# jayleicn/TVRetrieval

Hardware: AMD Instinct MI355X
Metric: queries/sec VCMR over 21.8K-video corpus (higher is better)
Workload: dtype bf16

## Files before the change

tvretrieval_amd/csrc/convse.hip:

```cpp
#include "band.h"
#include "gemm.h"

static constexpr int TM = 64;
static constexpr int LP = 128 + 8;
static constexpr int LH = 4;

static constexpr int CONVSE_SUB_MAX = 16;
static inline int convse_sub(int64_t P, int nv) { return P >= 128 * (int64_t)nv ? CONVSE_SUB_MAX : 1; }

struct ConvseWs {
  int32_t* counts;
  int32_t* offsets;
  int32_t* pos;
  int32_t* chunk_off;
  int32_t* bucket;
  int32_t* chunk_vid;
};

static size_t convse_ws_layout(const xml_convse_desc* d, ConvseWs* w, char* base) {
  size_t off = 0;
  auto take = [&](size_t bytes) {
    char* p = base ? base + off : nullptr;
    off += align_up(bytes, 256);
    return p;
  };
  const size_t nv = (size_t)d->nv, P = (size_t)d->nq * d->kpairs;
  char* counts = take(nv * CONVSE_SUB_MAX * 4);
  char* offsets = take((nv * CONVSE_SUB_MAX + 1) * 4);
  char* chunk_off = take((nv + 1) * 4);
  char* bucket = take(P * 4);
  char* pos = take(P * 4);
  char* chunk_vid = take((P / TM + (P < nv ? P : nv) + 1) * 4);
  if (w) {
    w->chunk_vid = (int32_t*)chunk_vid;
    w->counts = (int32_t*)counts; w->pos = (int32_t*)pos; w->offsets = (int32_t*)offsets;
    w->chunk_off = (int32_t*)chunk_off; w->bucket = (int32_t*)bucket;
  }
  return off;
}

extern "C" size_t xml_convse_rerank_workspace_bytes(const xml_convse_desc* d) {
  if (!d) return 0;
  return convse_ws_layout(d, nullptr, nullptr);
}

__global__ void convse_count_kernel(const int32_t* __restrict__ pair_vid, int32_t* __restrict__ counts,
                                    int32_t* __restrict__ pos, int64_t P, int nv, int sub) {
  const int64_t p = (int64_t)blockIdx.x * blockDim.x + threadIdx.x;
  if (p >= P) return;
  const int v = pair_vid[p];
  pos[p] = (v >= 0 && v < nv) ? atomicAdd(&counts[(int64_t)v * sub + (int)(p & (sub - 1))], 1) : -1;
}

__global__ void convse_zero_skipped_kernel(const int32_t* __restrict__ pair_vid, float* __restrict__ st_out,
                                           float* __restrict__ ed_out, int64_t P, int nv, int lpad4) {
  const int64_t p = (int64_t)blockIdx.x * blockDim.x + threadIdx.x;
  if (p >= P) return;
  const int v = pair_vid[p];
  if (v >= 0 && v < nv) return;
  const float4 z = make_float4(0.f, 0.f, 0.f, 0.f);
  float4* s4 = reinterpret_cast<float4*>(st_out) + p * lpad4;
  float4* e4 = reinterpret_cast<float4*>(ed_out) + p * lpad4;
  for (int i = 0; i < lpad4; ++i) { s4[i] = z; e4[i] = z; }
}

__global__ __launch_bounds__(1024) void convse_scan_kernel(const int32_t* __restrict__ counts,
                                                           int32_t* __restrict__ offsets,
                                                           int32_t* __restrict__ chunk_off,
                                                           int32_t* __restrict__ chunk_vid, int nv, int TM, int sub) {
  __shared__ int32_t wa[16], wb[16];
  const int tid = threadIdx.x, lane = tid & 63, wave = tid >> 6;
  const int per = (nv + 1023) / 1024;
  const int r0 = min(nv, tid * per), r1 = min(nv, r0 + per);
  int sa = 0, sb = 0;
  for (int i = r0; i < r1; ++i) {
    int c = 0;
    for (int j = 0; j < sub; ++j) c += counts[(int64_t)i * sub + j];
    sa += c; sb += (c + TM - 1) / TM;
  }
  int ia = sa, ib = sb;
#pragma unroll
  for (int o = 1; o < 64; o <<= 1) {
    const int va = __shfl_up(ia, o, 64), vb = __shfl_up(ib, o, 64);
    if (lane >= o) { ia += va; ib += vb; }
  }
  if (lane == 63) { wa[wave] = ia; wb[wave] = ib; }
  __syncthreads();
  int a = ia - sa, b = ib - sb;
  for (int w = 0; w < wave; ++w) { a += wa[w]; b += wb[w]; }
  for (int i = r0; i < r1; ++i) {
    int c = 0;
    for (int j = 0; j < sub; ++j) {
      const int cj = counts[(int64_t)i * sub + j];
      offsets[(int64_t)i * sub + j] = a + c;
      c += cj;
    }
    const int ch = (c + TM - 1) / TM;
    chunk_off[i] = b;
    for (int j = 0; j < ch; ++j) chunk_vid[b + j] = i;
    a += c; b += ch;
  }
  if (tid == 1023) { offsets[(int64_t)nv * sub] = a; chunk_off[nv] = b; }
}

__global__ void convse_fill_kernel(const int32_t* __restrict__ pair_vid, const int32_t* __restrict__ offsets,
                                   const int32_t* __restrict__ pos, int32_t* __restrict__ bucket, int64_t P, int sub) {
  const int64_t p = (int64_t)blockIdx.x * blockDim.x + threadIdx.x;
  if (p >= P) return;
  const int r = pos[p];
  if (r >= 0) bucket[offsets[(int64_t)pair_vid[p] * sub + (int)(p & (sub - 1))] + r] = (int32_t)p;
}

static constexpr int CONVSE_SMALL_NV = 4096, CONVSE_SMALL_P = 32768;
__global__ __launch_bounds__(1024) void convse_invert_small_kernel(const int32_t* __restrict__ pair_vid,
                                                                   int32_t* __restrict__ offsets, int32_t* __restrict__ chunk_off,
                                                                   int32_t* __restrict__ chunk_vid, int32_t* __restrict__ pos,
                                                                   int32_t* __restrict__ bucket, float* __restrict__ st_out,
                                                                   float* __restrict__ ed_out, int P, int nv, int TM, int lpad4,
                                                                   int zero_skipped) {
  __shared__ int32_t s_cnt[CONVSE_SMALL_NV], s_off[CONVSE_SMALL_NV];
  __shared__ int32_t wa[16], wb[16];
  const int tid = threadIdx.x, lane = tid & 63, wave = tid >> 6;
  for (int i = tid; i < nv; i += 1024) s_cnt[i] = 0;
  const bool in_regs = P <= 8 * 1024;
  int v_r[8], pos_r[8];
#pragma unroll
  for (int j = 0; j < 8; ++j) {
    const int p = tid + j * 1024;
    v_r[j] = (in_regs && p < P) ? pair_vid[p] : -1;
  }
  __syncthreads();
  if (in_regs) {
#pragma unroll
    for (int j = 0; j < 8; ++j) {
      const int p = tid + j * 1024;
      const bool ok = v_r[j] >= 0 && v_r[j] < nv;
      pos_r[j] = ok ? atomicAdd(&s_cnt[v_r[j]], 1) : -1;
      if (p < P && !ok && zero_skipped) {
        const float4 z = make_float4(0.f, 0.f, 0.f, 0.f);
        float4* s4 = reinterpret_cast<float4*>(st_out) + (int64_t)p * lpad4;
        float4* e4 = reinterpret_cast<float4*>(ed_out) + (int64_t)p * lpad4;
        for (int i = 0; i < lpad4; ++i) { s4[i] = z; e4[i] = z; }
      }
    }
  } else {
  for (int p = tid; p < P; p += 1024) {
    const int v = pair_vid[p];
    const bool ok = v >= 0 && v < nv;
    pos[p] = ok ? atomicAdd(&s_cnt[v], 1) : -1;
    if (!ok && zero_skipped) {
      const float4 z = make_float4(0.f, 0.f, 0.f, 0.f);
      float4* s4 = reinterpret_cast<float4*>(st_out) + (int64_t)p * lpad4;
      float4* e4 = reinterpret_cast<float4*>(ed_out) + (int64_t)p * lpad4;
      for (int i = 0; i < lpad4; ++i) { s4[i] = z; e4[i] = z; }
    }
  }
  }
  __syncthreads();
  const int per = (nv + 1023) / 1024;
  const int r0 = min(nv, tid * per), r1 = min(nv, r0 + per);
// ... 503 lines not shown
  if (d->n_mod < 1 || d->n_mod > 2 || (d->n_mod == 2 && (!q_lin1 || !feat2_1))) return XML_ERR_BAD_ARG;
  if (d->n_mod == 2 && !d->merged && !mask1) return XML_ERR_BAD_ARG;
  if (d->merged && d->n_mod != 2) return XML_ERR_BAD_ARG;
  if (d->lpad % 16 || d->lpad > 128 || d->l_ref > d->lpad || d->l_ref <= 0 || d->hidden % 8) return XML_ERR_UNSUPPORTED;
  if (!(d->ksize & 1) || d->ksize > 15 || d->ksize < 1) return XML_ERR_UNSUPPORTED;
  if (d->dt != XML_F32 && d->dt != XML_BF16) return XML_ERR_BAD_ARG;
  return convse_rerank_impl(d, q_lin0, q_lin1, feat2_0, feat2_1, mask0, mask1, pair_vid, conv_w, st_out, ed_out, ws, ws_bytes,
                            nullptr, nullptr, nullptr, nullptr, stream);
}

extern "C" int xml_convse_rerank_f16s(const xml_convse_desc* d, const void* q_lin0, const void* q_lin1, const float* q_inv0,
                                      const float* q_inv1, const void* feat2_0, const void* feat2_1, const float* c_inv0,
                                      const float* c_inv1, const float* mask0, const float* mask1, const int32_t* pair_vid,
                                      const float* conv_w, float* st_out, float* ed_out, void* ws, size_t ws_bytes,
                                      xml_stream_t stream) {
  XML_ENTER();
  if (!d || !q_lin0 || !feat2_0 || !mask0 || !pair_vid || !conv_w || !st_out || !ed_out || !ws || !q_inv0 || !c_inv0)
    return XML_ERR_BAD_ARG;
  if (d->nq <= 0 || d->nv <= 0 || d->kpairs <= 0 || d->hidden <= 0) return XML_ERR_BAD_ARG;
  if (d->n_mod < 1 || d->n_mod > 2 || (d->n_mod == 2 && (!q_lin1 || !feat2_1 || !q_inv1 || !c_inv1))) return XML_ERR_BAD_ARG;
  if (d->n_mod == 2 && !d->merged && !mask1) return XML_ERR_BAD_ARG;
  if (d->merged && d->n_mod != 2) return XML_ERR_BAD_ARG;
  if (d->lpad % 16 || d->lpad > 128 || d->l_ref > d->lpad || d->l_ref <= 0 || d->hidden % 32) return XML_ERR_UNSUPPORTED;
  if (!(d->ksize & 1) || d->ksize > 15 || d->ksize < 1) return XML_ERR_UNSUPPORTED;
  if (d->dt != XML_F16S) return XML_ERR_BAD_ARG;
  return convse_rerank_impl(d, q_lin0, q_lin1, feat2_0, feat2_1, mask0, mask1, pair_vid, conv_w, st_out, ed_out, ws, ws_bytes,
                            q_inv0, q_inv1, c_inv0, c_inv1, stream);
}

static int convse_rerank_impl(const xml_convse_desc* d, const void* q_lin0, const void* q_lin1, const void* feat2_0,
                              const void* feat2_1, const float* mask0, const float* mask1, const int32_t* pair_vid,
                              const float* conv_w, float* st_out, float* ed_out, void* ws, size_t ws_bytes,
                              const float* q_inv0, const float* q_inv1, const float* c_inv0, const float* c_inv1,
                              xml_stream_t stream, ConvseSumm sm, ConvseEv ev) {
  xml_convse_desc dl = *d;
  if (ev.pair_q) { dl.nq = (int)ev.n_pairs; dl.kpairs = 1; }
  if (!ev.pair_q && ws_bytes < xml_convse_rerank_workspace_bytes(d)) return XML_ERR_WORKSPACE;
  hipStream_t st = (hipStream_t)stream;
  ConvseWs w;
  convse_ws_layout(&dl, &w, (char*)ws);
  const int64_t P = (int64_t)dl.nq * dl.kpairs;
  int sub = 1;
  if (P <= CONVSE_SMALL_P && d->nv <= CONVSE_SMALL_NV) {
    hipLaunchKernelGGL(convse_invert_small_kernel, dim3(1), dim3(1024), 0, st, pair_vid, w.offsets, w.chunk_off, w.chunk_vid,
                       w.pos, w.bucket, st_out, ed_out, (int)P, d->nv, TM, d->lpad / 4, (d->softmax & 2) ? 0 : 1);
    XML_CHECK_LAUNCH();
  } else {
    {
      const int64_t nwords = (int64_t)((char*)w.offsets - (char*)w.counts) / 4;
      hipLaunchKernelGGL(convse_zero_words_kernel, dim3(cdiv(nwords, 256)), dim3(256), 0, st, (uint32_t*)w.counts, nwords);
      XML_CHECK_LAUNCH();
    }
    sub = convse_sub(P, d->nv);
    hipLaunchKernelGGL(convse_count_kernel, dim3(cdiv(P, 256)), dim3(256), 0, st, pair_vid, w.counts, w.pos, P, d->nv, sub);
    XML_CHECK_LAUNCH();
    if (!(d->softmax & 2)) {
      hipLaunchKernelGGL(convse_zero_skipped_kernel, dim3(cdiv(P, 256)), dim3(256), 0, st, pair_vid, st_out, ed_out, P,
                         d->nv, d->lpad / 4);
      XML_CHECK_LAUNCH();
    }
    hipLaunchKernelGGL(convse_scan_kernel, dim3(1), dim3(1024), 0, st, w.counts, w.offsets, w.chunk_off, w.chunk_vid,
                       d->nv, TM, sub);
    XML_CHECK_LAUNCH();
    hipLaunchKernelGGL(convse_fill_kernel, dim3(cdiv(P, 256)), dim3(256), 0, st, pair_vid, w.offsets, w.pos, w.bucket, P, sub);
    XML_CHECK_LAUNCH();
  }
  ConvseArgs a;
  a.sub = sub;
  a.q_lin[0] = q_lin0; a.q_lin[1] = q_lin1;
  a.feat2[0] = feat2_0; a.feat2[1] = feat2_1;
  a.mask[0] = mask0; a.mask[1] = mask1 ? mask1 : mask0;
  a.conv_w = conv_w; a.st_out = st_out; a.ed_out = ed_out;
  a.offsets = w.offsets; a.chunk_off = w.chunk_off; a.bucket = w.bucket; a.chunk_vid = w.chunk_vid;
  a.pair_q = ev.pair_q; a.ev_sim[0] = ev.sim[0]; a.ev_sim[1] = ev.sim[1]; a.ev_merged = ev.merged;
  a.nv = d->nv; a.kpairs = dl.kpairs; a.lpad = d->lpad; a.l_ref = d->l_ref; a.hidden = d->hidden;
  a.n_mod = d->n_mod; a.merged = d->merged; a.ksize = d->ksize; a.softmax = d->softmax & 1;
  a.dbg = g_q2c_ablation;
  a.pair_w = sm.pair_w; a.summ = sm.summ; a.min_l = sm.min_l; a.max_l = sm.max_l; a.vid_len = sm.vid_len;
  a.q_inv[0] = q_inv0; a.q_inv[1] = q_inv1 ? q_inv1 : q_inv0;
  a.c_inv[0] = c_inv0; a.c_inv[1] = c_inv1 ? c_inv1 : c_inv0;
  {
    const int64_t kb = (int64_t)d->hidden * (int64_t)dt_size(d->dt);
    a.dma = (kb % 128 == 0 && (int64_t)d->nq * kb < (1ll << 32) && (int64_t)d->lpad * kb < (1ll << 32)) ? 1 : 0;
    if (g_q2c_ablation == 40) a.dma = 0;
  }
  const int64_t max_chunks = P / TM + (P < d->nv ? P : d->nv);
  const int n_sim = d->merged ? 1 : d->n_mod;
  const size_t patch = (size_t)TM * LP * 4;
  if (d->dt == XML_F16S) {
    if (!a.dma) return XML_ERR_UNSUPPORTED;
    using Cfg = GemmCfg<f16s_t, TM, 128, 1, 4>;
    constexpr size_t stg = Cfg::LDS_BYTES;
    const size_t lds = n_sim == 1 ? (stg > patch ? stg : patch) : stg + 2 * patch;
    if (ev.pair_q) {
      if (!xml_lds_attr_once<convse_kernel<f16s_t, true>>((int)(stg + 2 * patch))) return XML_ERR_LAUNCH;
      hipLaunchKernelGGL((convse_kernel<f16s_t, true>), dim3((unsigned)max_chunks), dim3(256), lds, st, a);
    } else {
      if (!xml_lds_attr_once<convse_kernel<f16s_t>>((int)(stg + 2 * patch))) return XML_ERR_LAUNCH;
      hipLaunchKernelGGL(convse_kernel<f16s_t>, dim3((unsigned)max_chunks), dim3(256), lds, st, a);
    }
  } else if (d->dt == XML_F32) {
    using Cfg = GemmCfg<float, TM, 128, 1, 4>;
    constexpr size_t stg = Cfg::LDS_BYTES;
    const size_t lds = n_sim == 1 ? (stg > patch ? stg : patch) : stg + 2 * patch;
    if (ev.pair_q) {
      if (!xml_lds_attr_once<convse_kernel<float, true>>((int)(stg + 2 * patch))) return XML_ERR_LAUNCH;
      hipLaunchKernelGGL((convse_kernel<float, true>), dim3((unsigned)max_chunks), dim3(256), lds, st, a);
    } else {
      if (!xml_lds_attr_once<convse_kernel<float>>((int)(stg + 2 * patch))) return XML_ERR_LAUNCH;
      hipLaunchKernelGGL(convse_kernel<float>, dim3((unsigned)max_chunks), dim3(256), lds, st, a);
    }
  } else {
    using Cfg = GemmCfg<bf16_t, TM, 128, 1, 4>;
    constexpr size_t stg = Cfg::LDS_BYTES;
    const size_t lds = n_sim == 1 ? (stg > patch ? stg : patch) : stg + 2 * patch;
    if (ev.pair_q) {
      if (!xml_lds_attr_once<convse_kernel<bf16_t, true>>((int)(stg + 2 * patch))) return XML_ERR_LAUNCH;
// ... 53 lines not shown
  }
  size_t vid_off = 0;
  if (ws_bytes < evidence_ws_layout(d, n_pairs, &vid_off)) return XML_ERR_WORKSPACE;
  hipStream_t st = (hipStream_t)stream;
  int32_t* vid_ok = (int32_t*)((char*)ws + vid_off);
  hipLaunchKernelGGL(evidence_pairs_kernel, dim3(cdiv(n_pairs, 256)), dim3(256), 0, st, pair_q, pair_vid, vid_ok, n_pairs,
                     d->nq, d->nv);
  XML_CHECK_LAUNCH();
  hipLaunchKernelGGL(convse_zero_skipped_kernel, dim3(cdiv(n_pairs, 256)), dim3(256), 0, st, vid_ok, sim0_out, sim_out,
                     n_pairs, d->nv, d->lpad / 4);
  XML_CHECK_LAUNCH();
  if (d->n_mod == 2) {
    hipLaunchKernelGGL(convse_zero_skipped_kernel, dim3(cdiv(n_pairs, 256)), dim3(256), 0, st, vid_ok, sim1_out, sim1_out,
                       n_pairs, d->nv, d->lpad / 4);
    XML_CHECK_LAUNCH();
  }
  xml_convse_desc dd = *d;
  dd.softmax = 0;
  return convse_rerank_impl(&dd, q_lin0, q_lin1, feat2_0, feat2_1, mask0, mask1, vid_ok, conv_w, st_out, ed_out, ws, ws_bytes,
                            split ? q_inv0 : nullptr, split ? q_inv1 : nullptr, split ? c_inv0 : nullptr,
                            split ? c_inv1 : nullptr, stream, ConvseSumm{nullptr, nullptr, 0, 0, nullptr},
                            ConvseEv{pair_q, n_pairs, {sim0_out, d->n_mod == 2 ? sim1_out : nullptr}, sim_out});
}

extern "C" size_t xml_q2c_rescore_workspace_bytes(int nq, int nv, int kpairs) {
  xml_convse_desc d{};
  d.nq = nq; d.nv = nv; d.kpairs = kpairs;
  return convse_ws_layout(&d, nullptr, nullptr);
}

extern "C" int xml_q2c_rescore(int n_mod, const void* qn0, const void* qn1, const void* cn0, const void* cn1,
                               const float* mask0, const float* mask1, const int32_t* pair_vid, float* out, int nq, int nv,
                               int kpairs, int lpad, int hidden, int dt, void* ws, size_t ws_bytes, xml_stream_t stream) {
  XML_ENTER();
  if (!qn0 || !cn0 || !mask0 || !pair_vid || !out || !ws) return XML_ERR_BAD_ARG;
  if (n_mod < 1 || n_mod > 2 || (n_mod == 2 && (!qn1 || !cn1 || !mask1))) return XML_ERR_BAD_ARG;
  if (nq <= 0 || nv <= 0 || kpairs <= 0 || hidden <= 0) return XML_ERR_BAD_ARG;
  if (lpad % 16 || lpad > 128 || lpad <= 0 || hidden % 8) return XML_ERR_UNSUPPORTED;
  if (dt != XML_F32 && dt != XML_BF16 && dt != XML_F16S) return XML_ERR_BAD_ARG;
  if (dt == XML_F16S && hidden % 32) return XML_ERR_UNSUPPORTED;
  if (ws_bytes < xml_q2c_rescore_workspace_bytes(nq, nv, kpairs)) return XML_ERR_WORKSPACE;
  hipStream_t st = (hipStream_t)stream;
  xml_convse_desc d{};
  d.nq = nq; d.nv = nv; d.kpairs = kpairs;
  ConvseWs w;
  convse_ws_layout(&d, &w, (char*)ws);
  const int64_t P = (int64_t)nq * kpairs;
  {
    const int64_t nwords = (int64_t)((char*)w.offsets - (char*)w.counts) / 4;
    hipLaunchKernelGGL(convse_zero_words_kernel, dim3(cdiv(nwords, 256)), dim3(256), 0, st, (uint32_t*)w.counts, nwords);
    XML_CHECK_LAUNCH();
  }
  const int sub = convse_sub(P, nv);
  hipLaunchKernelGGL(convse_count_kernel, dim3(cdiv(P, 256)), dim3(256), 0, st, pair_vid, w.counts, w.pos, P, nv, sub);
  XML_CHECK_LAUNCH();
  hipLaunchKernelGGL(rescore_fill_skipped_kernel, dim3(cdiv(P, 256)), dim3(256), 0, st, pair_vid, out, P, nv);
  XML_CHECK_LAUNCH();
  const bool big = dt == XML_F16S && P > 64 * (int64_t)nv;
  hipLaunchKernelGGL(convse_scan_kernel, dim3(1), dim3(1024), 0, st, w.counts, w.offsets, w.chunk_off, w.chunk_vid, nv,
                     big ? 128 : TM, sub);
  XML_CHECK_LAUNCH();
  hipLaunchKernelGGL(convse_fill_kernel, dim3(cdiv(P, 256)), dim3(256), 0, st, pair_vid, w.offsets, w.pos, w.bucket, P, sub);
  XML_CHECK_LAUNCH();
  RescoreArgs a;
  a.sub = sub;
  a.qn[0] = qn0; a.qn[1] = qn1; a.cn[0] = cn0; a.cn[1] = cn1;
  a.mask[0] = mask0; a.mask[1] = mask1 ? mask1 : mask0;
  a.out = out;
  a.offsets = w.offsets; a.chunk_off = w.chunk_off; a.bucket = w.bucket; a.chunk_vid = w.chunk_vid;
  a.nv = nv; a.kpairs = kpairs; a.lpad = lpad; a.hidden = hidden; a.n_mod = n_mod;
  {
    const int64_t kb = (int64_t)hidden * (int64_t)dt_size(dt);
    a.dma = (kb % 128 == 0 && (int64_t)nq * kb < (1ll << 32) && (int64_t)lpad * kb < (1ll << 32)) ? 1 : 0;
    if (g_q2c_ablation == 40) a.dma = 0;
  }
  const int64_t max_chunks = P / TM + (P < nv ? P : nv);
  if (dt == XML_F16S && big) {
    if (!a.dma) return XML_ERR_UNSUPPORTED;
    using Cfg = GemmCfg<f16s_t, 128, 128, 1, 4>;
    constexpr int lds = GemmDma<Cfg, RS_STAGES>::LDS_BYTES;
    if (!xml_lds_attr_once<rescore_kernel<f16s_t, 128>>(lds)) return XML_ERR_LAUNCH;
    const int64_t chunks128 = P / 128 + (P < nv ? P : nv);
    hipLaunchKernelGGL((rescore_kernel<f16s_t, 128>), dim3((unsigned)chunks128), dim3(256), lds, st, a);
  } else if (dt == XML_F16S) {
    using Cfg = GemmCfg<f16s_t, TM, 128, 1, 4>;
    constexpr int lds = GemmDma<Cfg, RS_STAGES>::LDS_BYTES;
    if (!xml_lds_attr_once<rescore_kernel<f16s_t>>(lds)) return XML_ERR_LAUNCH;
    hipLaunchKernelGGL(rescore_kernel<f16s_t>, dim3((unsigned)max_chunks), dim3(256), lds, st, a);
  } else if (dt == XML_F32) {
    using Cfg = GemmCfg<float, TM, 128, 1, 4>;
    constexpr int lds = GemmDma<Cfg, RS_STAGES>::LDS_BYTES;
    if (!xml_lds_attr_once<rescore_kernel<float>>(lds)) return XML_ERR_LAUNCH;
    hipLaunchKernelGGL(rescore_kernel<float>, dim3((unsigned)max_chunks), dim3(256), lds, st, a);
  } else {
    using Cfg = GemmCfg<bf16_t, TM, 128, 1, 4>;
    constexpr int lds = GemmDma<Cfg, RS_STAGES>::LDS_BYTES;
    if (!xml_lds_attr_once<rescore_kernel<bf16_t>>(lds)) return XML_ERR_LAUNCH;
    hipLaunchKernelGGL(rescore_kernel<bf16_t>, dim3((unsigned)max_chunks), dim3(256), lds, st, a);
  }
  XML_CHECK_LAUNCH();
  return XML_OK;
}
```

tvretrieval_amd/csrc/linear.hip:

```cpp
#include "gemm.h"
#include "internal.h"
#include "l2norm.h"

template <typename T, typename OutT, typename AddT, int BMN = 128>
__global__ __launch_bounds__(256) void gemm_bias_act_kernel(const T* __restrict__ A, const T* __restrict__ W,
                                                            const float* __restrict__ bias,
                                                            const AddT* __restrict__ addend, OutT* __restrict__ out,
                                                            int64_t M, int N, int K, int relu, int add_mode,
                                                            int seq_len, const float* __restrict__ row_scale) {
  using Cfg = GemmCfg<T, BMN, BMN, 2, 2>;
  __shared__ __attribute__((aligned(16))) char smem[Cfg::LDS_BYTES];
  const int64_t m0 = (int64_t)blockIdx.y * Cfg::BM;
  const int n0 = blockIdx.x * Cfg::BN;
  f32x4 acc[Cfg::MT][Cfg::NT];
  auto a_row = [&](int r) -> const char* {
    const int64_t m = m0 + r;
    return m < M ? reinterpret_cast<const char*>(A + m * K) : nullptr;
  };
  auto b_row = [&](int r) -> const char* {
    const int n = n0 + r;
    return n < N ? reinterpret_cast<const char*>(W + (int64_t)n * K) : nullptr;
  };
  if constexpr (BMN < 128 && !IsSplit16<T>::value && !std::is_same<T, f16_t>::value) {
    const int nsteps = (K * (int)sizeof(T) + Cfg::ROWB - 1) / Cfg::ROWB;
// ... 421 lines not shown

extern "C" int xml_linear_add(const void* x, const void* w, const float* b, const void* addend, void* y, int64_t rows, int n,
                              int k, int relu, int dt, xml_stream_t stream) {
  XML_ENTER();
  if (!x || !w || !y || !addend) return XML_ERR_BAD_ARG;
  if (dt != XML_F32 && dt != XML_BF16) return XML_ERR_UNSUPPORTED;
  return xmli_gemm(x, w, b, addend, y, rows, n, k, relu, 2, 1, 0, dt, (hipStream_t)stream);
}

extern "C" size_t xml_linear_f16s_workspace_bytes(int64_t rows, int k) { return xmli_gemm_split_ws_bytes(rows, k, XML_F16S); }
extern "C" int xml_linear_f16s(const float* x, const void* w, const float* b, float* y, int64_t rows, int n, int k, int relu,
                               void* ws, size_t ws_bytes, xml_stream_t stream) {
  XML_ENTER();
  if (!x || !w || !y || !ws) return XML_ERR_BAD_ARG;
  if (rows > 0 && ws_bytes < xmli_gemm_split_ws_bytes(rows, k, XML_F16S)) return XML_ERR_WORKSPACE;
  return xmli_gemm(x, w, b, nullptr, y, rows, n, k, relu, 0, 1, 1, XML_F16S, (hipStream_t)stream, ws);
}

static inline int k_pad8(int d_in) { return (d_in + 7) & ~7; }
extern "C" size_t xml_linear_ln_relu_pos_workspace_bytes(int64_t rows, int d_in, int hidden, int dt) {
  const size_t pre = align_up((size_t)rows * hidden * 4, 256);
  const size_t lnw = xmli_gemm_ln_eligible(rows, hidden, k_pad8(d_in), dt) ? xmli_gemm_ln_workspace_bytes(rows, hidden) : 0;
  return align_up((size_t)rows * k_pad8(d_in) * dt_size(dt), 256) + (pre > lnw ? pre : lnw) +
         xmli_gemm_split_ws_bytes(rows, k_pad8(d_in), dt);
}

extern "C" int xml_linear_ln_relu_pos(const void* x, int x_dt, const float* ln_in_g, const float* ln_in_b,
                                      const void* w, const float* b, const void* pos, const float* ln_pos_g,
                                      const float* ln_pos_b, void* y, int64_t rows, int seq_len, int d_in, int hidden,
                                      int dt, void* ws, size_t ws_bytes, xml_stream_t stream) {
  XML_ENTER();
  if (!x || !ln_in_g || !ln_in_b || !w || !b || !pos || !ln_pos_g || !ln_pos_b || !y || !ws) return XML_ERR_BAD_ARG;
  if (rows <= 0 || seq_len <= 0 || !xmli_model_dt_ok(dt)) return XML_ERR_BAD_ARG;
  if (d_in <= 0 || hidden % 8) return XML_ERR_UNSUPPORTED;
  if (ws_bytes < xml_linear_ln_relu_pos_workspace_bytes(rows, d_in, hidden, dt)) return XML_ERR_WORKSPACE;
  hipStream_t st = (hipStream_t)stream;
  const int d_pad = k_pad8(d_in);
  const int adt = xmli_act_dt(dt);
  char* xn = (char*)ws;
  char* pre = xn + align_up((size_t)rows * d_pad * dt_size(dt), 256);
  char* sws = dt == XML_F16S ? (char*)ws + xml_linear_ln_relu_pos_workspace_bytes(rows, d_in, hidden, dt) -
                                   xmli_gemm_split_ws_bytes(rows, d_pad, dt) : nullptr;
  int rc = xmli_add_layernorm(x, x_dt, nullptr, ln_in_g, ln_in_b, xn, rows, d_in, d_pad, adt, st);
  if (rc) return rc;
  if (xmli_gemm_ln_eligible(rows, hidden, d_pad, dt) &&
      xmli_gemm_ln(xn, w, b, pos, ln_pos_g, ln_pos_b, y, rows, hidden, d_pad,  1,  1, seq_len, dt, pre,
                   st) == XML_OK)
    return XML_OK;
  rc = xmli_gemm(xn, w, b, pos, pre, rows, hidden, d_pad,  1,  1, seq_len,  1, dt, st, sws);
  if (rc) return rc;
  return xmli_gemm_ln_tail((const float*)pre, ln_pos_g, ln_pos_b, y, rows, hidden, dt, st);
}

__global__ __launch_bounds__(256) void pack_len_kernel(const float* __restrict__ mask, int n, int lq, int32_t* __restrict__ cu,
                                                       int32_t* __restrict__ status) {
  const int lane = threadIdx.x & 63;
  const int r = blockIdx.x * 4 + (threadIdx.x >> 6);
  if (r >= n) return;
  const float v = lane < lq ? mask[(int64_t)r * lq + lane] : 0.f;
  const unsigned long long ones = __ballot(v == 1.f), other = __ballot(v != 1.f && v != 0.f);
  const int len = (int)__popcll(ones);
  const bool ok = other == 0 && len > 0 && ones == (len == 64 ? ~0ull : ((1ull << len) - 1ull));
  if (lane == 0) {
    cu[r + 1] = len;
    if (!ok) atomicOr(&status[1], 1);
  }
}

__global__ __launch_bounds__(1024) void pack_scan_kernel(int n, int32_t* __restrict__ cu, int32_t* __restrict__ status) {
  __shared__ int s_wave[16];
  const int tid = threadIdx.x, lane = tid & 63, wave = tid >> 6;
  const int per = (n + 1023) / 1024;
  const int r0 = min(n, tid * per), r1 = min(n, r0 + per);
  int sum = 0;
  for (int r = r0; r < r1; ++r) sum += cu[r + 1];
  int inc = sum;
#pragma unroll
  for (int o = 1; o < 64; o <<= 1) {
    const int v = __shfl_up(inc, o, 64);
    if (lane >= o) inc += v;
  }
  if (lane == 63) s_wave[wave] = inc;
  __syncthreads();
  int base = inc - sum;
  for (int w = 0; w < wave; ++w) base += s_wave[w];
  for (int r = r0; r < r1; ++r) {
    base += cu[r + 1];
    cu[r + 1] = base;
  }
  if (tid == 0) {
    cu[0] = 0;
    int total = 0;
    for (int w = 0; w < 16; ++w) total += s_wave[w];
    status[0] = status[1] ? -1 : total;
  }
}

__global__ __launch_bounds__(256) void pack_fill_kernel(int n, int lq, const int32_t* __restrict__ cu, int32_t* __restrict__ src_row) {
  const int lane = threadIdx.x & 63;
  const int r = blockIdx.x * 4 + (threadIdx.x >> 6);
  if (r >= n) return;
  const int b = cu[r], len = cu[r + 1] - b;
  if (lane < len) src_row[b + lane] = r * lq + lane;
}

extern "C" int xml_pack_plan(const float* mask, int64_t n, int lq, int32_t* cu_seqlens, int32_t* src_row, int32_t* status,
                             xml_stream_t stream) {
  XML_ENTER();
  if (!mask || !cu_seqlens || !src_row || !status || n <= 0 || lq <= 0) return XML_ERR_BAD_ARG;
  if (lq > 64 || n * lq > (int64_t)INT32_MAX) return XML_ERR_UNSUPPORTED;
  hipStream_t st = (hipStream_t)stream;
  xml_zero_async(status, 8, st);
  hipLaunchKernelGGL(pack_len_kernel, dim3(cdiv(n, 4)), dim3(256), 0, st, mask, (int)n, lq, cu_seqlens, status);
  hipLaunchKernelGGL(pack_scan_kernel, dim3(1), dim3(1024), 0, st, (int)n, cu_seqlens, status);
  hipLaunchKernelGGL(pack_fill_kernel, dim3(cdiv(n, 4)), dim3(256), 0, st, (int)n, lq, cu_seqlens, src_row);
  XML_CHECK_LAUNCH();
  return XML_OK;
}

__global__ __launch_bounds__(256) void gather_pos_rows_kernel(const uint4* __restrict__ table, const int32_t* __restrict__ src_row,
                                                              uint4* __restrict__ dst, int64_t rows, int lq, int vec_per_row) {
  const int64_t i = (int64_t)blockIdx.x * 256 + threadIdx.x;
  if (i >= rows * vec_per_row) return;
  const int64_t r = i / vec_per_row;
  const int v = (int)(i - r * vec_per_row);
  dst[i] = table[(int64_t)(src_row[r] % lq) * vec_per_row + v];
}

extern "C" size_t xml_linear_ln_relu_pos_packed_workspace_bytes(int64_t rows, int d_in, int hidden, int dt) {
  return xml_linear_ln_relu_pos_workspace_bytes(rows, d_in, hidden, dt) + align_up((size_t)rows * hidden * dt_size(dt), 256);
}

extern "C" int xml_linear_ln_relu_pos_packed(const void* x, int x_dt, const int32_t* src_row, int lq, const float* ln_in_g,
                                             const float* ln_in_b, const void* w, const float* b, const void* pos,
                                             const float* ln_pos_g, const float* ln_pos_b, void* y, int64_t rows, int d_in,
                                             int hidden, int dt, void* ws, size_t ws_bytes, xml_stream_t stream) {
  XML_ENTER();
  if (!x || !src_row || !ln_in_g || !ln_in_b || !w || !b || !pos || !ln_pos_g || !ln_pos_b || !y || !ws) return XML_ERR_BAD_ARG;
  if (rows <= 0 || rows > (int64_t)INT32_MAX || lq <= 0 || !xmli_model_dt_ok(dt)) return XML_ERR_BAD_ARG;
  if (d_in <= 0 || d_in % 8 || d_in > 4096 || hidden % 8) return XML_ERR_UNSUPPORTED;
  if (ws_bytes < xml_linear_ln_relu_pos_packed_workspace_bytes(rows, d_in, hidden, dt)) return XML_ERR_WORKSPACE;
  hipStream_t st = (hipStream_t)stream;
  const int adt = xmli_act_dt(dt);
  char* pg = (char*)ws;
  char* xn = pg + align_up((size_t)rows * hidden * dt_size(dt), 256);
  char* pre = xn + align_up((size_t)rows * d_in * dt_size(dt), 256);
  char* sws = dt == XML_F16S ? (char*)ws + xml_linear_ln_relu_pos_packed_workspace_bytes(rows, d_in, hidden, dt) -
                                   xmli_gemm_split_ws_bytes(rows, d_in, dt) : nullptr;
  const int vpr = hidden * (int)dt_size(dt) / 16;
  hipLaunchKernelGGL(gather_pos_rows_kernel, dim3(cdiv(rows * vpr, 256)), dim3(256), 0, st, (const uint4*)pos, src_row,
                     (uint4*)pg, rows, lq, vpr);
  XML_CHECK_LAUNCH();
  int rc = add_layernorm_rows(x, x_dt, nullptr, ln_in_g, ln_in_b, xn, rows, d_in, d_in, adt, st, src_row);
  if (rc) return rc;
  if (xmli_gemm_ln_eligible(rows, hidden, d_in, dt) &&
      xmli_gemm_ln(xn, w, b, pg, ln_pos_g, ln_pos_b, y, rows, hidden, d_in,  1,  1, (int)rows, dt, pre,
                   st) == XML_OK)
    return XML_OK;
  rc = xmli_gemm(xn, w, b, pg, pre, rows, hidden, d_in,  1,  1, (int)rows,  1, dt, st, sws);
  if (rc) return rc;
  return xmli_gemm_ln_tail((const float*)pre, ln_pos_g, ln_pos_b, y, rows, hidden, dt, st);
}
```

tvretrieval_amd/csrc/topk.hip:

```cpp
#include "common.h"

__device__ __forceinline__ uint32_t ord_key(float f) {
  uint32_t u = __float_as_uint(f);
  if (u == 0x80000000u) u = 0u;
  return (u & 0x80000000u) ? ~u : (u | 0x80000000u);
}
__device__ __forceinline__ float key_to_float(uint32_t k) {
  return __uint_as_float((k & 0x80000000u) ? (k & 0x7fffffffu) : ~k);
}

template <bool ALLOW>
struct TopkAllow {};
template <>
struct TopkAllow<true> {
  const uint32_t* bits;
  int64_t ld;
  int rows;
  int col0;
  int32_t* out_cnt;
};

template <int VPT, bool ALLOW = false>
__global__ __launch_bounds__(256) void topk_rows_kernel(const float* __restrict__ scores, int64_t ld,
                                                        const int32_t* __restrict__ idx_in,
// ... 32 lines not shown
    const uint32_t lo = col0, hi = col0 + (uint32_t)n, hs = col0 + (uint32_t)n_reg;
    uint32_t c_n = 0, c_s = 0;
    for (uint32_t w = (lo >> 5) + (uint32_t)tid; w <= ((hi - 1) >> 5); w += 256) {
      uint32_t v = arow[w];
      if (w == (lo >> 5)) v &= 0xffffffffu << (lo & 31u);
      uint32_t vs = v;
      if (w == ((hi - 1) >> 5) && (hi & 31u)) v &= 0xffffffffu >> (32u - (hi & 31u));
      if (w > ((hs - 1) >> 5)) vs = 0u;
      else if (w == ((hs - 1) >> 5) && (hs & 31u)) vs &= 0xffffffffu >> (32u - (hs & 31u));
      c_n += (uint32_t)__popc(v);
      c_s += (uint32_t)__popc(vs);
    }
    if (c_n) atomicAdd(&s_an, c_n);
    if (c_s) atomicAdd(&s_as, c_s);
    __syncthreads();
    a_n = s_an;
    a_s = s_as;
    k_sel = min((uint32_t)k, a_n);
    if (tid == 0 && aw.out_cnt) aw.out_cnt[blockIdx.x] = (int32_t)k_sel;
    if (k_sel == 0) {
      if (tid < k) {
        out_val[(int64_t)blockIdx.x * k + tid] = (alpha != 0.f) ? 0.f : -INFINITY;
        out_idx[(int64_t)blockIdx.x * k + tid] = -1;
      }
      return;
    }
  }
  uint32_t keys[NK];
  {
    float raw[NK];
    uint32_t abit[ALLOW ? NK : 1];
#pragma unroll
    for (int j = 0; j < NK; ++j) {
      const int i = tid + j * 256;
      raw[j] = i < n_reg ? row[i] : 0.f;
      if constexpr (ALLOW) abit[j] = i < n_reg ? arow[(col0 + (uint32_t)i) >> 5] : 0u;
    }
#pragma unroll
    for (int j = 0; j < NK; ++j) {
      keys[j] = tid + j * 256 < n_reg ? ord_key(raw[j]) : 0u;
      if constexpr (ALLOW) {
        if (!bit_of(abit[j], tid + j * 256)) keys[j] = 0u;
      }
    }
  }
  enum { SRC_REG = 0, SRC_ROW = 1, SRC_CAND = 2 };
  int src = VPT > 0 ? SRC_REG : SRC_ROW;
  int n_cand = 0;
  auto walk = [&](auto&& f) {
    if (src == SRC_REG) {
#pragma unroll
      for (int j = 0; j < NK; ++j) f(keys[j], tid + j * 256, ALLOW ? keys[j] != 0u : tid + j * 256 < n_reg);
    } else if (src == SRC_ROW) {
      for (int base = 0; base < n; base += 256 * 8) {
        float raw[8];
        uint32_t abit[ALLOW ? 8 : 1];
#pragma unroll
        for (int u = 0; u < 8; ++u) {
          const int i = base + u * 256 + tid;
          raw[u] = i < n ? row[i] : 0.f;
          if constexpr (ALLOW) abit[u] = i < n ? arow[(col0 + (uint32_t)i) >> 5] : 0u;
        }
#pragma unroll
        for (int u = 0; u < 8; ++u) {
          const int i = base + u * 256 + tid;
          if constexpr (ALLOW) {
            const bool ok = i < n && bit_of(abit[u], i);
            if (base + u * 256 < n) f(ok ? ord_key(raw[u]) : 0u, i, ok);
          } else {
            if (base + u * 256 < n) f(i < n ? ord_key(raw[u]) : 0u, i, i < n);
          }
        }
      }
    } else {
      for (int base = 0; base < n_cand; base += 256) {
        const int i = base + tid;
        const unsigned long long e = i < n_cand ? cand[i] : 0ull;
        f((uint32_t)(e >> 32), (int)(uint32_t)(e & 0xffffffffull), i < n_cand);
      }
    }
  };
  auto hist_pass = [&](uint32_t mask, uint32_t prefix, int shift) {
    walk([&](uint32_t key, int, bool valid) {
      const bool act = valid && (key & mask) == prefix;
      const uint32_t bin = (key >> shift) & 0xff;
      if (shift == 24) {
        unsigned long long todo = __ballot(act);
#pragma unroll 1
        for (int r = 0; r < 4 && todo; ++r) {
          const int leader = __ffsll((long long)todo) - 1;
          const uint32_t lb = __shfl(bin, leader, 64);
          const unsigned long long same = __ballot(act && bin == lb) & todo;
          if (lane == leader) atomicAdd(&hist[lb], (uint32_t)__popcll(same));
          todo &= ~same;
        }
        if ((todo >> lane) & 1ull) atomicAdd(&hist[bin], 1u);
      } else if (act) {
        atomicAdd(&hist[bin], 1u);
      }
    });
  };
  auto select = [&](uint32_t kth) {
    if (tid == 0) { s_prefix = 0; s_need = kth; }
    uint32_t mask = 0;
    for (int pass = 0; pass < 4; ++pass) {
      const int shift = 24 - 8 * pass;
      hist[tid] = 0;
      __syncthreads();
      const uint32_t prefix = s_prefix;
      hist_pass(mask, prefix, shift);
      __syncthreads();
      {
        const uint32_t need = s_need;
        const uint32_t h = hist[255 - tid];
        uint32_t inc = h;
#pragma unroll
        for (int o = 1; o < 64; o <<= 1) {
          const uint32_t v = __shfl_up(inc, o, 64);
          if (lane >= o) inc += v;
        }
        if (lane == 63) s_wsum[wave] = inc;
        __syncthreads();
        for (int w = 0; w < wave; ++w) inc += s_wsum[w];
        if (inc >= need && inc - h < need) {
          s_need = need - (inc - h);
// ... 182 lines not shown
```

Before: 145,800.

## Fuse convse zeroing into count, parallelize scan, vectorize topk row walk

Moves the zeroing of skipped pairs into the count kernel and the chunk_vid fill into the fill kernel, which removes a launch and the serial per-thread chunk_vid writes. The scan kernel is rewritten as a tiled block scan that stages results in shared memory so the global writes are coalesced. The pack length kernel now encodes bad rows in a flag bit, so the status zeroing memset and the atomic are no longer needed. The topk row path switches to float4 loads with separate handling for an unaligned head and a tail. Together these cut launch overhead and improve memory access, at the cost of more complex kernels and extra shared memory in the scan.

```diff
diff --git a/tvretrieval_amd/csrc/convse.hip b/tvretrieval_amd/csrc/convse.hip
--- a/tvretrieval_amd/csrc/convse.hip
+++ b/tvretrieval_amd/csrc/convse.hip
@@ -45,11 +45,19 @@
 }
 
 __global__ void convse_count_kernel(const int32_t* __restrict__ pair_vid, int32_t* __restrict__ counts,
-                                    int32_t* __restrict__ pos, int64_t P, int nv, int sub) {
+                                    int32_t* __restrict__ pos, int64_t P, int nv, int sub, float* __restrict__ st_out,
+                                    float* __restrict__ ed_out, int lpad4) {
   const int64_t p = (int64_t)blockIdx.x * blockDim.x + threadIdx.x;
   if (p >= P) return;
   const int v = pair_vid[p];
-  pos[p] = (v >= 0 && v < nv) ? atomicAdd(&counts[(int64_t)v * sub + (int)(p & (sub - 1))], 1) : -1;
+  const bool ok = v >= 0 && v < nv;
+  pos[p] = ok ? atomicAdd(&counts[(int64_t)v * sub + (int)(p & (sub - 1))], 1) : -1;
+  if (!ok && st_out) {
+    const float4 z = make_float4(0.f, 0.f, 0.f, 0.f);
+    float4* s4 = reinterpret_cast<float4*>(st_out) + p * lpad4;
+    float4* e4 = reinterpret_cast<float4*>(ed_out) + p * lpad4;
+    for (int i = 0; i < lpad4; ++i) { s4[i] = z; e4[i] = z; }
+  }
 }
 
 __global__ void convse_zero_skipped_kernel(const int32_t* __restrict__ pair_vid, float* __restrict__ st_out,
@@ -64,10 +72,83 @@
   for (int i = 0; i < lpad4; ++i) { s4[i] = z; e4[i] = z; }
 }
 
+static constexpr int SCAN_V = 4;
 __global__ __launch_bounds__(1024) void convse_scan_kernel(const int32_t* __restrict__ counts,
                                                            int32_t* __restrict__ offsets,
-                                                           int32_t* __restrict__ chunk_off,
-                                                           int32_t* __restrict__ chunk_vid, int nv, int TM, int sub) {
+                                                           int32_t* __restrict__ chunk_off, int nv, int TM, int sub) {
+  __shared__ int32_t wa[2][16], wb[2][16];
+  __shared__ int32_t s_off[1024 * SCAN_V], s_cho[1024 * SCAN_V];
+  const int tid = threadIdx.x, lane = tid & 63, wave = tid >> 6;
+  auto load_tile = [&](int base, int (&c)[SCAN_V]) {
+#pragma unroll
+    for (int u = 0; u < SCAN_V; ++u) {
+      const int i = base + tid * SCAN_V + u;
+      c[u] = 0;
+      if (i < nv) {
+        if (sub == 1) c[u] = counts[i];
+        else for (int j = 0; j < sub; ++j) c[u] += counts[(int64_t)i * sub + j];
+      }
+    }
+  };
+  int carry_a = 0, carry_b = 0;
+  int c[SCAN_V], cn[SCAN_V];
+  load_tile(0, c);
+  for (int base = 0, t = 0; base < nv; base += 1024 * SCAN_V, t ^= 1) {
+    load_tile(base + 1024 * SCAN_V, cn);
+    int ch[SCAN_V];
+    int sa = 0, sb = 0;
+#pragma unroll
+    for (int u = 0; u < SCAN_V; ++u) { ch[u] = (c[u] + TM - 1) / TM; sa += c[u]; sb += ch[u]; }
+    int ia = sa, ib = sb;
+#pragma unroll
+    for (int o = 1; o < 64; o <<= 1) {
+      const int va = __shfl_up(ia, o, 64), vb = __shfl_up(ib, o, 64);
+      if (lane >= o) { ia += va; ib += vb; }
+    }
+    if (lane == 63) { wa[t][wave] = ia; wb[t][wave] = ib; }
+    __syncthreads();
+    int a = carry_a + ia - sa, b = carry_b + ib - sb;
+#pragma unroll
+    for (int w = 0; w < 16; ++w) {
+      const int xa = wa[t][w], xb = wb[t][w];
+      if (w < wave) { a += xa; b += xb; }
+      carry_a += xa; carry_b += xb;
+    }
+#pragma unroll
+    for (int u = 0; u < SCAN_V; ++u) {
+      const int i = base + tid * SCAN_V + u;
+      s_off[tid * SCAN_V + u] = a;
+      s_cho[tid * SCAN_V + u] = b;
+      if (sub != 1 && i < nv) {
+        int cc = 0;
+        for (int j = 0; j < sub; ++j) {
+          const int cj = counts[(int64_t)i * sub + j];
+          offsets[(int64_t)i * sub + j] = a + cc;
+          cc += cj;
+        }
+      }
+      a += c[u]; b += ch[u];
+    }
+    __syncthreads();
+#pragma unroll
+    for (int r = 0; r < SCAN_V; ++r) {
+      const int e = r * 1024 + tid, i = base + e;
+      if (i < nv) {
+        if (sub == 1) offsets[i] = s_off[e];
+        chunk_off[i] = s_cho[e];
+      }
+    }
+#pragma unroll
+    for (int u = 0; u < SCAN_V; ++u) c[u] = cn[u];
+  }
+  if (tid == 0) { offsets[(int64_t)nv * sub] = carry_a; chunk_off[nv] = carry_b; }
+}
+
+#ifdef XML_DEBUG_VARIANTS
+__global__ __launch_bounds__(1024) void convse_scan_serial_kernel(const int32_t* __restrict__ counts,
+                                                                  int32_t* __restrict__ offsets,
+                                                                  int32_t* __restrict__ chunk_off,
+                                                                  int32_t* __restrict__ chunk_vid, int nv, int TM, int sub) {
   __shared__ int32_t wa[16], wb[16];
   const int tid = threadIdx.x, lane = tid & 63, wave = tid >> 6;
   const int per = (nv + 1023) / 1024;
@@ -102,10 +183,16 @@
   }
   if (tid == 1023) { offsets[(int64_t)nv * sub] = a; chunk_off[nv] = b; }
 }
+#endif
 
 __global__ void convse_fill_kernel(const int32_t* __restrict__ pair_vid, const int32_t* __restrict__ offsets,
-                                   const int32_t* __restrict__ pos, int32_t* __restrict__ bucket, int64_t P, int sub) {
+                                   const int32_t* __restrict__ pos, int32_t* __restrict__ bucket, int64_t P, int sub,
+                                   const int32_t* __restrict__ chunk_off, int32_t* __restrict__ chunk_vid, int nv) {
   const int64_t p = (int64_t)blockIdx.x * blockDim.x + threadIdx.x;
+  if (chunk_vid && p < nv) {
+    const int b1 = chunk_off[p + 1];
+    for (int b = chunk_off[p]; b < b1; ++b) chunk_vid[b] = (int32_t)p;
+  }
   if (p >= P) return;
   const int r = pos[p];
   if (r >= 0) bucket[offsets[(int64_t)pair_vid[p] * sub + (int)(p & (sub - 1))] + r] = (int32_t)p;
@@ -715,17 +802,30 @@
       XML_CHECK_LAUNCH();
     }
     sub = convse_sub(P, d->nv);
-    hipLaunchKernelGGL(convse_count_kernel, dim3(cdiv(P, 256)), dim3(256), 0, st, pair_vid, w.counts, w.pos, P, d->nv, sub);
+    const bool zero_skipped = !(d->softmax & 2);
+    bool parent_inversion = false;
+#ifdef XML_DEBUG_VARIANTS
+    parent_inversion = g_q2c_ablation == 42;
+#endif
+    hipLaunchKernelGGL(convse_count_kernel, dim3(cdiv(P, 256)), dim3(256), 0, st, pair_vid, w.counts, w.pos, P, d->nv, sub,
+                       zero_skipped && !parent_inversion ? st_out : nullptr, ed_out, d->lpad / 4);
     XML_CHECK_LAUNCH();
-    if (!(d->softmax & 2)) {
-      hipLaunchKernelGGL(convse_zero_skipped_kernel, dim3(cdiv(P, 256)), dim3(256), 0, st, pair_vid, st_out, ed_out, P,
-                         d->nv, d->lpad / 4);
-      XML_CHECK_LAUNCH();
-    }
-    hipLaunchKernelGGL(convse_scan_kernel, dim3(1), dim3(1024), 0, st, w.counts, w.offsets, w.chunk_off, w.chunk_vid,
-                       d->nv, TM, sub);
+#ifdef XML_DEBUG_VARIANTS
+    if (parent_inversion) {
+      if (zero_skipped) {
+        hipLaunchKernelGGL(convse_zero_skipped_kernel, dim3(cdiv(P, 256)), dim3(256), 0, st, pair_vid, st_out, ed_out, P,
+                           d->nv, d->lpad / 4);
+        XML_CHECK_LAUNCH();
+      }
+      hipLaunchKernelGGL(convse_scan_serial_kernel, dim3(1), dim3(1024), 0, st, w.counts, w.offsets, w.chunk_off,
+                         w.chunk_vid, d->nv, TM, sub);
+    } else
+#endif
+    hipLaunchKernelGGL(convse_scan_kernel, dim3(1), dim3(1024), 0, st, w.counts, w.offsets, w.chunk_off, d->nv, TM, sub);
     XML_CHECK_LAUNCH();
-    hipLaunchKernelGGL(convse_fill_kernel, dim3(cdiv(P, 256)), dim3(256), 0, st, pair_vid, w.offsets, w.pos, w.bucket, P, sub);
+    const int64_t n_fill = P > d->nv ? P : (int64_t)d->nv;
+    hipLaunchKernelGGL(convse_fill_kernel, dim3(cdiv(n_fill, 256)), dim3(256), 0, st, pair_vid, w.offsets, w.pos, w.bucket, P,
+                       sub, w.chunk_off, parent_inversion ? nullptr : w.chunk_vid, d->nv);
     XML_CHECK_LAUNCH();
   }
   ConvseArgs a;
@@ -885,15 +985,18 @@
     XML_CHECK_LAUNCH();
   }
   const int sub = convse_sub(P, nv);
-  hipLaunchKernelGGL(convse_count_kernel, dim3(cdiv(P, 256)), dim3(256), 0, st, pair_vid, w.counts, w.pos, P, nv, sub);
+  hipLaunchKernelGGL(convse_count_kernel, dim3(cdiv(P, 256)), dim3(256), 0, st, pair_vid, w.counts, w.pos, P, nv, sub,
+                     (float*)nullptr, (float*)nullptr, 0);
   XML_CHECK_LAUNCH();
   hipLaunchKernelGGL(rescore_fill_skipped_kernel, dim3(cdiv(P, 256)), dim3(256), 0, st, pair_vid, out, P, nv);
   XML_CHECK_LAUNCH();
   const bool big = dt == XML_F16S && P > 64 * (int64_t)nv;
-  hipLaunchKernelGGL(convse_scan_kernel, dim3(1), dim3(1024), 0, st, w.counts, w.offsets, w.chunk_off, w.chunk_vid, nv,
-                     big ? 128 : TM, sub);
+  hipLaunchKernelGGL(convse_scan_kernel, dim3(1), dim3(1024), 0, st, w.counts, w.offsets, w.chunk_off, nv, big ? 128 : TM,
+                     sub);
   XML_CHECK_LAUNCH();
-  hipLaunchKernelGGL(convse_fill_kernel, dim3(cdiv(P, 256)), dim3(256), 0, st, pair_vid, w.offsets, w.pos, w.bucket, P, sub);
+  const int64_t n_fill = P > nv ? P : (int64_t)nv;
+  hipLaunchKernelGGL(convse_fill_kernel, dim3(cdiv(n_fill, 256)), dim3(256), 0, st, pair_vid, w.offsets, w.pos, w.bucket, P, sub,
+                     w.chunk_off, w.chunk_vid, nv);
   XML_CHECK_LAUNCH();
   RescoreArgs a;
   a.sub = sub;
diff --git a/tvretrieval_amd/csrc/linear.hip b/tvretrieval_amd/csrc/linear.hip
--- a/tvretrieval_amd/csrc/linear.hip
+++ b/tvretrieval_amd/csrc/linear.hip
@@ -497,8 +497,8 @@
   return xmli_gemm_ln_tail((const float*)pre, ln_pos_g, ln_pos_b, y, rows, hidden, dt, st);
 }
 
-__global__ __launch_bounds__(256) void pack_len_kernel(const float* __restrict__ mask, int n, int lq, int32_t* __restrict__ cu,
-                                                       int32_t* __restrict__ status) {
+static constexpr int32_t PACK_BAD = 1 << 30;
+__global__ __launch_bounds__(256) void pack_len_kernel(const float* __restrict__ mask, int n, int lq, int32_t* __restrict__ cu) {
   const int lane = threadIdx.x & 63;
   const int r = blockIdx.x * 4 + (threadIdx.x >> 6);
   if (r >= n) return;
@@ -506,38 +506,41 @@
   const unsigned long long ones = __ballot(v == 1.f), other = __ballot(v != 1.f && v != 0.f);
   const int len = (int)__popcll(ones);
   const bool ok = other == 0 && len > 0 && ones == (len == 64 ? ~0ull : ((1ull << len) - 1ull));
-  if (lane == 0) {
-    cu[r + 1] = len;
-    if (!ok) atomicOr(&status[1], 1);
-  }
+  if (lane == 0) cu[r + 1] = ok ? len : (len | PACK_BAD);
 }
 
 __global__ __launch_bounds__(1024) void pack_scan_kernel(int n, int32_t* __restrict__ cu, int32_t* __restrict__ status) {
-  __shared__ int s_wave[16];
+  __shared__ int s_wave[16], s_bad[16];
   const int tid = threadIdx.x, lane = tid & 63, wave = tid >> 6;
   const int per = (n + 1023) / 1024;
   const int r0 = min(n, tid * per), r1 = min(n, r0 + per);
-  int sum = 0;
-  for (int r = r0; r < r1; ++r) sum += cu[r + 1];
+  int sum = 0, bad = 0;
+  for (int r = r0; r < r1; ++r) {
+    const int v = cu[r + 1];
+    sum += v & (PACK_BAD - 1);
+    bad |= v & PACK_BAD;
+  }
+  bad = __any(bad);
   int inc = sum;
 #pragma unroll
   for (int o = 1; o < 64; o <<= 1) {
     const int v = __shfl_up(inc, o, 64);
     if (lane >= o) inc += v;
   }
-  if (lane == 63) s_wave[wave] = inc;
+  if (lane == 63) { s_wave[wave] = inc; s_bad[wave] = bad; }
   __syncthreads();
   int base = inc - sum;
   for (int w = 0; w < wave; ++w) base += s_wave[w];
   for (int r = r0; r < r1; ++r) {
-    base += cu[r + 1];
+    base += cu[r + 1] & (PACK_BAD - 1);
     cu[r + 1] = base;
   }
   if (tid == 0) {
     cu[0] = 0;
-    int total = 0;
-    for (int w = 0; w < 16; ++w) total += s_wave[w];
-    status[0] = status[1] ? -1 : total;
+    int total = 0, any_bad = 0;
+    for (int w = 0; w < 16; ++w) { total += s_wave[w]; any_bad |= s_bad[w]; }
+    status[1] = any_bad ? 1 : 0;
+    status[0] = any_bad ? -1 : total;
   }
 }
 
@@ -555,8 +558,7 @@
   if (!mask || !cu_seqlens || !src_row || !status || n <= 0 || lq <= 0) return XML_ERR_BAD_ARG;
   if (lq > 64 || n * lq > (int64_t)INT32_MAX) return XML_ERR_UNSUPPORTED;
   hipStream_t st = (hipStream_t)stream;
-  xml_zero_async(status, 8, st);
-  hipLaunchKernelGGL(pack_len_kernel, dim3(cdiv(n, 4)), dim3(256), 0, st, mask, (int)n, lq, cu_seqlens, status);
+  hipLaunchKernelGGL(pack_len_kernel, dim3(cdiv(n, 4)), dim3(256), 0, st, mask, (int)n, lq, cu_seqlens);
   hipLaunchKernelGGL(pack_scan_kernel, dim3(1), dim3(1024), 0, st, (int)n, cu_seqlens, status);
   hipLaunchKernelGGL(pack_fill_kernel, dim3(cdiv(n, 4)), dim3(256), 0, st, (int)n, lq, cu_seqlens, src_row);
   XML_CHECK_LAUNCH();
diff --git a/tvretrieval_amd/csrc/topk.hip b/tvretrieval_amd/csrc/topk.hip
--- a/tvretrieval_amd/csrc/topk.hip
+++ b/tvretrieval_amd/csrc/topk.hip
@@ -108,25 +108,45 @@
 #pragma unroll
       for (int j = 0; j < NK; ++j) f(keys[j], tid + j * 256, ALLOW ? keys[j] != 0u : tid + j * 256 < n_reg);
     } else if (src == SRC_ROW) {
-      for (int base = 0; base < n; base += 256 * 8) {
-        float raw[8];
-        uint32_t abit[ALLOW ? 8 : 1];
-#pragma unroll
-        for (int u = 0; u < 8; ++u) {
-          const int i = base + u * 256 + tid;
-          raw[u] = i < n ? row[i] : 0.f;
-          if constexpr (ALLOW) abit[u] = i < n ? arow[(col0 + (uint32_t)i) >> 5] : 0u;
-        }
-#pragma unroll
-        for (int u = 0; u < 8; ++u) {
-          const int i = base + u * 256 + tid;
+      constexpr int RU = ALLOW ? 4 : 8;
+      const int head = min(n, (int)(((16u - (uint32_t)(reinterpret_cast<uintptr_t>(row) & 15u)) & 15u) >> 2));
+      const int nvec = (n - head) >> 2, tail0 = head + 4 * nvec;
+      const float4* row4 = reinterpret_cast<const float4*>(row + head);
+      for (int base = 0; base < nvec; base += 256 * RU) {
+        float4 raw[RU];
+        uint32_t abit[ALLOW ? RU : 1][ALLOW ? 4 : 1];
+#pragma unroll
+        for (int u = 0; u < RU; ++u) {
+          const int v = base + u * 256 + tid;
+          raw[u] = v < nvec ? row4[v] : make_float4(0.f, 0.f, 0.f, 0.f);
           if constexpr (ALLOW) {
-            const bool ok = i < n && bit_of(abit[u], i);
-            if (base + u * 256 < n) f(ok ? ord_key(raw[u]) : 0u, i, ok);
-          } else {
-            if (base + u * 256 < n) f(i < n ? ord_key(raw[u]) : 0u, i, i < n);
+#pragma unroll
+            for (int c = 0; c < 4; ++c) abit[u][c] = v < nvec ? arow[(col0 + (uint32_t)(head + 4 * v + c)) >> 5] : 0u;
           }
         }
+#pragma unroll
+        for (int u = 0; u < RU; ++u) {
+          const int v = base + u * 256 + tid;
+          if (base + u * 256 >= nvec) continue;
+          const float x[4] = {raw[u].x, raw[u].y, raw[u].z, raw[u].w};
+#pragma unroll
+          for (int c = 0; c < 4; ++c) {
+            const int i = head + 4 * v + c;
+            bool ok = v < nvec;
+            if constexpr (ALLOW) ok = ok && bit_of(abit[u][c], i);
+            f(ok ? ord_key(x[c]) : 0u, i, ok);
+          }
+        }
+      }
+      {
+        const int i = tid < head ? tid : tail0 + (tid - head);
+        bool ok = i < n && tid < 8;
+        uint32_t key = 0u;
+        if (ok) {
+          if constexpr (ALLOW) ok = bit_of(arow[(col0 + (uint32_t)i) >> 5], i);
+          if (ok) key = ord_key(row[i]);
+        }
+        if (wave == 0) f(key, i, ok);
       }
     } else {
       for (int base = 0; base < n_cand; base += 256) {
```

New measurement: 145,800 (median of 2 runs). No clear change (+0.0%).
